# injun-baek/Video-Depth-Normal-v2

Measured on AMD Instinct MI355X. Metric: depth frames/sec at 518x518, ViT-L, higher is better.
Workload: dtype f16x3; 1 GPU; DepthAnythingV2(vitl) batch=8 518x518 streams/GPU, memory bank full (S=6); replicas per GPU; lanes=2, precision=f16x3, ranks=1, backend=none, attention_pv_products=1

## Files before the change

### include/vdn.h

```cpp
#ifndef VDN_H
#define VDN_H
#include <stddef.h>
#include <stdint.h>

#ifdef __cplusplus
extern "C" {
#endif

typedef void* vdn_stream;

enum vdn_status { VDN_OK = 0, VDN_EINVAL = -1, VDN_EUNSUPPORTED = -2, VDN_EALIGN = -3 };
enum vdn_dtype { VDN_F16 = 0, VDN_BF16 = 1, VDN_F32 = 2, VDN_NONE = 3 };
enum vdn_act { VDN_ACT_NONE = 0, VDN_ACT_GELU = 1, VDN_ACT_RELU = 2,
               VDN_ACT_SILU = 3  };
enum vdn_amode { VDN_A_PLAIN = 0, VDN_A_CONV3X3 = 1 };
enum vdn_store {
  VDN_ST_PLAIN = 0,
  VDN_ST_HEADS = 1,
  VDN_ST_CONVT = 2,
  VDN_ST_GEGLU = 3
};

typedef struct vdn_gemm_tuning {
  int force_bm;
  int p8;
  int no_splitk;
  int no_pipe;
  int splitk_p8;
  int cus;
  int splitk_occ;
  int splitk_max;
  int min_tiles;
  float f128, f192;
  int x8;
} vdn_gemm_tuning;
int vdn_gemm_get_tuning(vdn_gemm_tuning* out);

typedef struct vdn_gemm_desc {
  int32_t dt;
  int32_t M, N, K;
  const void* A;
  int32_t a_mode;
  int32_t lda;
  int32_t relu_a;
  int32_t cB, cH, cW, cC, cOH, cOW, cstride;
  const void* W;
  int32_t ldb;
  const float* bias;
  const float* rowadd;
  int32_t act;
  const float* gamma;
  const float* tab;
  int32_t tab_mod, tab_off;
  const void* res1;
  int32_t res1_dt, ldr1;
  const void* res2;
  int32_t res2_dt, ldr2;
  int32_t store;
  void* out;
  int32_t out_dt;
  int32_t ldc;
  int32_t row_group, row_skip;
  void* dst[3];
  int32_t nsplit, heads, tokens, tok_off, tpad;
  int32_t transposed[3];
  int32_t rope[3];
  const float* rope_cs;
  int32_t rope_mod;
  int32_t ck, cout;
  const void* zeros;
  const void* A_lo;
  const void* W_lo;
  void* out_lo;
  void* dst_lo[3];
  const void* res1_lo;
  const void* res2_lo;
  int32_t conv_korder;
  int32_t cu_hint;
  void* splitk_ws;
  int64_t splitk_ws_bytes;
  int32_t ksplit;
  void* dst8[3];
  const void* A8;
  const void* W8;
  void* out8;
  int32_t a_kt, w_kt, out_kt;
  int32_t x8_terms;
// ... 196 lines not shown
```

### video-depth-normal-v2_amd/csrc/common.hpp

```cpp
#pragma once
#include <hip/hip_runtime.h>
#include <stdint.h>
#include <type_traits>
#include "../../include/vdn.h"

typedef _Float16 f16x8 __attribute__((ext_vector_type(8)));
typedef _Float16 f16x4 __attribute__((ext_vector_type(4)));
typedef _Float16 f16x2 __attribute__((ext_vector_type(2)));
typedef __bf16 bf16x8 __attribute__((ext_vector_type(8)));
typedef __bf16 bf16x4 __attribute__((ext_vector_type(4)));
typedef __bf16 bf16x2 __attribute__((ext_vector_type(2)));
typedef float f32x2 __attribute__((ext_vector_type(2)));
typedef float f32x4 __attribute__((ext_vector_type(4)));
typedef float f32x16 __attribute__((ext_vector_type(16)));
typedef uint32_t u32x4 __attribute__((ext_vector_type(4)));
typedef uint32_t u32x2 __attribute__((ext_vector_type(2)));

#define VDN_CHECK_LAUNCH()                                   \
  do {                                                       \
    hipError_t e__ = hipGetLastError();                      \
    if (e__ != hipSuccess) return -(1000 + (int)e__);        \
  } while (0)

template <int DT> struct Half;
// ... 156 lines not shown
}
constexpr float VDN_LO8_SCALE = 1024.0f;
constexpr int VDN_LO8_E8M0 = 117;

typedef _Float16 f16x32 __attribute__((ext_vector_type(32)));
typedef unsigned u32x6 __attribute__((ext_vector_type(6)));
__device__ __forceinline__ int x6_scale_byte(const f16x32& hi) {
  typedef unsigned short u16x32 __attribute__((ext_vector_type(32)));
  typedef unsigned short u16x16 __attribute__((ext_vector_type(16)));
  typedef unsigned short u16x8 __attribute__((ext_vector_type(8)));
  typedef unsigned short u16x4 __attribute__((ext_vector_type(4)));
  typedef unsigned short u16x2 __attribute__((ext_vector_type(2)));
  const u16x32 b = __builtin_bit_cast(u16x32, hi) & (unsigned short)0x7FFF;
  const u16x16 m16 = __builtin_elementwise_max(b.lo, b.hi);
  const u16x8 m8 = __builtin_elementwise_max(m16.lo, m16.hi);
  const u16x4 m4 = __builtin_elementwise_max(m8.lo, m8.hi);
  const u16x2 m2 = __builtin_elementwise_max(m4.lo, m4.hi);
  const unsigned m = m2[0] > m2[1] ? m2[0] : m2[1];
  return (int)(m >> 10) + 108;
}
__device__ __forceinline__ void x6_store_half(uint8_t* dst, const f16x32& v, int scale_byte) {
  const u32x6 c = __builtin_amdgcn_cvt_scalef32_pk32_bf6_f16(v, __builtin_bit_cast(float, (unsigned)scale_byte << 23));
  *(u32x4*)dst = u32x4{c[0], c[1], c[2], c[3]};
  *(u32x4*)(dst + 16) = u32x4{c[4], c[5], (unsigned)scale_byte, 0u};
}
__host__ __device__ __forceinline__ int x6_col(int order, int h, int p) {
  return order == 1 ? 32 * (p >> 4) + 16 * ((p >> 3) & 1) + 8 * h + (p & 7)
       : order == 2 ? 32 * (p >> 4) + 8 * ((p >> 2) & 3) + 4 * h + (p & 3)
                    : 32 * h + p;
}

template <typename T>
__device__ __forceinline__ void store_half(T* hi, T* lo, size_t i, float v) {
  if (lo) { T a, b; split_rtz(v, a, b); hi[i] = a; lo[i] = b; }
  else hi[i] = (T)v;
}
template <typename T>
__device__ __forceinline__ void store_half_nearest(T* hi, T* lo, size_t i, float v) {
  const T a = (T)v;
  hi[i] = a;
  if (lo) lo[i] = (T)(v - (float)a);
}
template <typename T>
__device__ __forceinline__ float load_half(const T* hi, const T* lo, size_t i) {
  return lo ? (float)hi[i] + (float)lo[i] : (float)hi[i];
}

__device__ __forceinline__ int xcd_remap(int orig, int nwg) {
  const int xcd = orig & 7;
  const int q = nwg >> 3, r = nwg & 7;
  const int base = (xcd < r) ? xcd * (q + 1) : r * (q + 1) + (xcd - r) * q;
  return base + (orig >> 3);
}
```

### video-depth-normal-v2_amd/csrc/gemm.hip

```cpp
#include "common.hpp"
#include <stdlib.h>

namespace vdn_gemm_impl {
int launch_f16(const vdn_gemm_desc& d, hipStream_t s);
int launch_bf16(const vdn_gemm_desc& d, hipStream_t s);

static int env_int(const char* name, int dflt) {
  const char* e = getenv(name);
  return e ? atoi(e) : dflt;
}
static float env_float(const char* name, float dflt) {
  const char* e = getenv(name);
  return e ? (float)atof(e) : dflt;
}
static const vdn_gemm_tuning& tuning_defaults() {
  static const vdn_gemm_tuning t = [] {
    vdn_gemm_tuning v;
    v.force_bm = env_int("VDN_GEMM_BM", 0);
    v.p8 = env_int("VDN_GEMM_P8", 1);
    v.no_splitk = getenv("VDN_GEMM_NOSPLITK") != nullptr;
    v.no_pipe = getenv("VDN_GEMM_NOPIPE") != nullptr;
    v.splitk_p8 = env_int("VDN_SPLITK_P8", 0);
    v.cus = env_int("VDN_GEMM_CUS", 0);
    v.splitk_occ = env_int("VDN_SPLITK_OCC", 50);
    v.splitk_max = env_int("VDN_SPLITK_MAX", 8);
    v.min_tiles = env_int("VDN_GEMM_MIN_TILES", 96);
    v.f128 = env_float("VDN_GEMM_F128", 1.3f);
    v.f192 = env_float("VDN_GEMM_F192", 1.2f);
    v.x8 = env_int("VDN_GEMM_X8", 1);
    return v;
  }();
  return t;
}
const vdn_gemm_tuning& tuning(const vdn_gemm_desc& d) { return d.tuning ? *d.tuning : tuning_defaults(); }
}

extern "C" int vdn_gemm_get_tuning(vdn_gemm_tuning* out) {
  if (!out) return VDN_EINVAL;
  vdn_gemm_desc none = {};
  *out = vdn_gemm_impl::tuning(none);
  return VDN_OK;
}

extern "C" int vdn_gemm(const vdn_gemm_desc* dp, vdn_stream stream) {
  if (!dp) return VDN_EINVAL;
  const vdn_gemm_desc& d = *dp;
  if (d.M <= 0 || d.N <= 0 || d.K <= 0 || !d.A || !d.W || !d.zeros) return VDN_EINVAL;
  if (d.tuning) {
    const vdn_gemm_tuning& t = *d.tuning;
    if ((t.force_bm != 0 && t.force_bm != 128 && t.force_bm != 192 && t.force_bm != 256) || t.splitk_occ < 0 || t.splitk_max < 0 ||
        t.min_tiles < 0 || t.cus < 0 || t.cus > 256)
      return VDN_EINVAL;
  }
  if (d.dt != VDN_F16 && d.dt != VDN_BF16) return VDN_EUNSUPPORTED;
  if ((d.K & 7) || (d.ldb & 63) || d.ldb < d.K) return VDN_EALIGN;
  if (((uintptr_t)d.A & 15) || ((uintptr_t)d.W & 15) || ((uintptr_t)d.zeros & 15)) return VDN_EALIGN;
  if (d.subpix) {
    if (d.subpix != 1 || d.a_mode != VDN_A_CONV3X3 || d.store != VDN_ST_CONVT || !d.subpix_bias || d.bias || d.act || d.rowadd ||
        d.gamma || d.tab || d.res1 || d.res2 || d.relu_a || d.K != 4 * d.cC || d.ldb != d.K || d.conv_korder != 1 || d.cstride != 1)
      return VDN_EINVAL;
    if ((d.ck != 2 && d.ck != 4) || d.cout <= 0 || (d.cout & 255) || (d.cC & 63) || !d.A_lo || !d.W_lo || !d.out_lo ||
        d.out_dt != d.dt || d.A8 || d.W8)
      return VDN_EUNSUPPORTED;
    if (((uintptr_t)d.subpix_bias | (uintptr_t)d.out) & 15) return VDN_EALIGN;
  }
  if (d.a_mode == VDN_A_CONV3X3) {
    if ((d.cC & 7) || d.K != (d.subpix ? 4 : 9) * d.cC || d.M != d.cB * d.cOH * d.cOW) return VDN_EINVAL;
    if (d.conv_korder && ((d.cC & 63) || d.conv_korder != 1)) return VDN_EINVAL;
    if (d.cstride != 1 && d.cstride != 2) return VDN_EUNSUPPORTED;
    if (d.cOH != (d.cH + 2 - 3) / d.cstride + 1 || d.cOW != (d.cW + 2 - 3) / d.cstride + 1) return VDN_EINVAL;
  } else if (d.a_mode == VDN_A_PLAIN) {
    if ((d.lda & 7) || d.lda < d.K) return VDN_EALIGN;
  } else {
    return VDN_EUNSUPPORTED;
  }
  if (d.N & 3) return VDN_EALIGN;
  if (d.ksplit != 0 || d.splitk_ws_bytes < 0 || (d.splitk_ws == nullptr) != (d.splitk_ws_bytes == 0)) return VDN_EINVAL;
  if ((uintptr_t)d.splitk_ws & 15) return VDN_EALIGN;
  if (((uintptr_t)d.A_lo | (uintptr_t)d.W_lo | (uintptr_t)d.out_lo) & 15) return VDN_EALIGN;
  if (d.out_lo && (d.out_dt == VDN_F32 || !d.out)) return VDN_EINVAL;
  if ((d.res1 && (d.ldr1 & 3)) || (d.res2 && (d.ldr2 & 3))) return VDN_EALIGN;
  if (((uintptr_t)d.A8 | (uintptr_t)d.W8 | (uintptr_t)d.out8) & 15) return VDN_EALIGN;
  if ((d.A8 || d.W8) && (d.dt != VDN_F16 || d.a_mode != VDN_A_PLAIN || (d.K & 63) || (d.lda != d.K && !d.a_kt))) return VDN_EINVAL;
  if (d.out8 && (d.dt != VDN_F16 || d.store != VDN_ST_PLAIN || d.out_dt != VDN_F16 || d.act != VDN_ACT_GELU || d.N != d.ldc || (d.N & 63) || !d.A8 || !d.W8))
    return VDN_EINVAL;
  if ((d.a_kt || d.w_kt || d.out_kt || d.x8_terms) && (!d.A8 || !d.W8)) return VDN_EINVAL;
  if (d.A8 && d.W8 && ((!d.a_kt && (long)d.M * d.lda >= (1L << 31)) || (!d.w_kt && (long)d.N * d.ldb >= (1L << 31)) || d.M >= (1 << 25) || d.N >= (1 << 25)))
    return VDN_EUNSUPPORTED;
  if (d.x8_terms < 0 || d.x8_terms > 2) return VDN_EINVAL;
  if (d.out_kt && (d.store != VDN_ST_PLAIN || d.out_dt != VDN_F16 || d.ldc != d.N || (d.N & 63) || d.res1 || d.res2 || d.tab ||
                   d.rowadd || d.gamma || d.row_group > 0 || d.act == VDN_ACT_RELU)) return VDN_EINVAL;
  if (((uintptr_t)d.bias | (uintptr_t)d.gamma | (uintptr_t)d.tab | (uintptr_t)d.res1 | (uintptr_t)d.res2) & 7) return VDN_EALIGN;
  switch (d.store) {
    case VDN_ST_PLAIN:
      if (!d.out || d.ldc < d.N) return VDN_EINVAL;
      if ((d.ldc & 3) || ((uintptr_t)d.out & 15)) return VDN_EALIGN;
      break;
    case VDN_ST_GEGLU:
      if (!d.out || (d.N & 31) || d.ldc < d.N / 2 || (d.act && d.act != VDN_ACT_SILU) || d.gamma || d.res1 || d.res2 || d.tab || d.rowadd)
        return VDN_EINVAL;
      if ((d.ldc & 3) || ((uintptr_t)d.out & 15)) return VDN_EALIGN;
      break;
    case VDN_ST_CONVT:
      if (!d.out || d.ck <= 0 || d.cout <= 0 || d.N != d.ck * d.ck * d.cout || d.M != d.cB * d.cH * d.cW || d.res1 ||
// ... 22 lines not shown
```

### video-depth-normal-v2_amd/csrc/gemm_kernels.hpp

```cpp
#pragma once
#include "common.hpp"
#include <stdlib.h>
#include <type_traits>

namespace vdn_gemm_impl {

const vdn_gemm_tuning& tuning(const vdn_gemm_desc& d);

constexpr int BK = 64;


__device__ __forceinline__ void glds16(const void* src, void* dst) {
  __builtin_amdgcn_global_load_lds((const __attribute__((address_space(1))) void*)src, (__attribute__((address_space(3))) void*)dst,
                                   16, 0, 0);
}

__device__ __forceinline__ void tile_mn(int tile, int tiles_m, int tiles_n, int& tm_i, int& tn_i) {
  constexpr int GM = 4;
  const int per_group = GM * tiles_n;
  const int g = tile / per_group, r = tile - g * per_group;
  const int gm = (tiles_m - g * GM) < GM ? (tiles_m - g * GM) : GM;
  tn_i = r / gm;
  tm_i = g * GM + (r - tn_i * gm);
}
// ... 939 lines not shown
      const int cur = kt & 1;
      const char* sc = smem + cur * STAGE;
      const char* sn = smem + (cur ^ 1) * STAGE;
      read_a(sc, 1, a1h, a1l);
      mma(0, a0h, a0l, bch, bcl);
      stage_barrier();
      if (kt + 2 < nk) issue(cur, kt + 2);
      if (kt + 1 < nk) {
        read_b(sn, bnh, bnl);
        read_a(sn, 0, a0h, a0l);
      }
      mma(1, a1h, a1l, bch, bcl);
    };
    int kt = 0;
    for (; kt + 1 < nk; kt += 2) {
      pstep(kt, b0h, b0l, b1h, b1l);
      pstep(kt + 1, b1h, b1l, b0h, b0l);
    }
    if (kt < nk) pstep(kt, b0h, b0l, b1h, b1l);
    stage_barrier();
  }

  epilogue_x3<DT, TMW, STORE>(acc, p, slice, m0 + wm * (BM / 2), n0 + wn * 64, lane);
}

template <int DT, int AMODE, int STORE, int BM>
__global__ __launch_bounds__(512) void gemm_x3_p8_kernel(const vdn_gemm_desc p) {
  using H = Half<DT>;
  using V8 = typename H::V8;
  using T = typename H::T;
  static_assert(BM == 256 || BM == 192, "A sub-halves of 64 or 48 rows");
  constexpr int BN = 256, BK3 = 32;
  constexpr int A_TILE = BM * 64, W_TILE = BN * 64;
  constexpr int STAGE = 2 * A_TILE + 2 * W_TILE;
  constexpr int TQ = BM / 64;
  constexpr bool CONV = (AMODE == 1 || AMODE == 2);
  constexpr bool RELU_A = (AMODE == 2 || AMODE == 3);
  extern __shared__ __attribute__((aligned(16))) char smem[];

  const int tid = threadIdx.x, lane = tid & 63;
  const int wave = __builtin_amdgcn_readfirstlane(tid >> 6);
  const int tiles_n = (p.N + BN - 1) / BN;
  const int tiles_m = (p.M + BM - 1) / BM;
  const int ntiles = tiles_m * tiles_n;
  constexpr bool SPLITK = STORE == VDN_STX_SPLITK;
  const int slice = SPLITK ? (int)blockIdx.x / ntiles : 0;
  const bool persistent = !SPLITK && (int)gridDim.x < ntiles;
  for (int it = 0;; ++it) {
  int tile;
  if constexpr (SPLITK) {
    if (it) break;
    tile = xcd_remap((int)blockIdx.x - slice * ntiles, ntiles);
  } else if (persistent) {
    const int xcd = blockIdx.x & 7, q8 = ntiles >> 3, r8 = ntiles & 7;
    const int base = xcd < r8 ? xcd * (q8 + 1) : r8 * (q8 + 1) + (xcd - r8) * q8;
    const int idx = (int)(blockIdx.x >> 3) + it * (int)(gridDim.x >> 3);
    if (idx >= q8 + (xcd < r8 ? 1 : 0)) break;
    tile = base + idx;
  } else {
    if (it) break;
    tile = xcd_remap(blockIdx.x, ntiles);
  }
  int tm_i, tn_i;
  tile_mn(tile, tiles_m, tiles_n, tm_i, tn_i);
  constexpr bool SUBPIX = STORE == VDN_STX_SUBPIX;
  unsigned sp_taps = 0;
  int sp_lg = 0;
  const int m0 = tm_i * BM, n0 = SUBPIX ? subpix_tile(tn_i, p, sp_taps, sp_lg) : tn_i * BN;
  const int wm = wave >> 2, wn = wave & 3;

  const int kt0s = SPLITK ? slice * ((((AMODE == 1 || AMODE == 2) ? p.ldb / BK3 : p.K / BK3) + p.ksplit - 1) / p.ksplit) : 0;
  const int lr = lane >> 2;
  const int chunk = (lane & 3) ^ ((0 - (lane >> 4)) & 3);
  const int a_li = (BM == 256 || wave < 4) ? wave : 4 + ((wave - 4) >> 1);
  const bool a_both = BM == 256 || wave < 4;
  const int a_plane = a_both ? 0 : (wave & 1);
  const int pa[2] = {(a_li / TQ) * 2 * TQ + a_li % TQ, (a_li / TQ) * 2 * TQ + TQ + a_li % TQ};
  const int pw[2] = {4 * (wave >> 1) + (wave & 1), 4 * (wave >> 1) + (wave & 1) + 2};
  APiece<T, CONV> a_pc[2];
#pragma unroll
  for (int i = 0; i < 2; ++i) a_pc[i].setup(m0 + pa[i] * 16 + lr, chunk * 8, p);
  const char* zeros = (const char*)p.zeros;
  const ptrdiff_t a_delta = (const char*)p.A_lo - (const char*)p.A;
  const ptrdiff_t w_delta = (const char*)p.W_lo - (const char*)p.W;
  const char* ap[2];
  const char* wp[2];
#pragma unroll
  for (int i = 0; i < 2; ++i) {
    int n = n0 + (vdn_pair8<STORE> ? (pw[i] >> 2) * 64 + pair8_col(pw[i] & 3, lr) : pw[i] * 16 + lr);
    n = n < p.N ? n : p.N - 1;
    wp[i] = (const char*)((const T*)p.W + (size_t)n * p.ldb + chunk * 8);
    ap[i] = (const char*)(a_pc[i].base + chunk * 8);
  }
  auto issue = [&](auto uc, int buf, int kt) {
    constexpr int u = decltype(uc)::value;
    char* s0 = smem + buf * STAGE;
    if constexpr (u == 0 || u == 3) {
      constexpr int i = u == 0 ? 0 : 1;
      char* dst = s0 + pa[i] * 1024;
      if constexpr (CONV) {
        bool ok;
        const char* src = a_pc[i].src(kstep_decode<BK3, SUBPIX>(kt + kt0s, p, sp_taps, sp_lg), chunk * 8, p, ok);
        if (a_both) {
          glds16(ok ? src : zeros, dst);
          glds16(ok ? src + a_delta : zeros, dst + A_TILE);
        } else {
          glds16(ok ? src + (a_plane ? a_delta : 0) : zeros, dst + a_plane * A_TILE);
        }
      } else {
        if (a_both) {
          glds16(ap[i], dst);
// ... 305 lines not shown
```

### video-depth-normal-v2_amd/csrc/gemm_x8.hip

```cpp
#include "gemm_kernels.hpp"

namespace vdn_gemm_impl {

typedef int i32x8 __attribute__((ext_vector_type(8)));

constexpr int X8_BN = 256;
constexpr int X8_WH = 256 * 64;
#ifndef VDN_X8_NSLOT
#define VDN_X8_NSLOT 5
#endif
#ifndef VDN_X8_ABL
#define VDN_X8_ABL 0
#endif
constexpr int X8_NSLOT = VDN_X8_NSLOT;
constexpr int x8_unit(int bm) { return bm * 64 + X8_WH; }
constexpr int X8_L = X8_NSLOT - 1;
constexpr int x8_pc(int ph, bool four) {
  const int a = four ? 2 : 1, w = 2;
  return a + w;
}
constexpr int x8_inflight(int newest, int k, bool four) {
  int n = 0;
  for (int t = 0; t < k; ++t) n += x8_pc((newest - t) & 3, four);
  return n;
}

template <int STORE, bool PAIR, int X8_BM>
__global__ __launch_bounds__(512) void gemm_x8_kernel(const vdn_gemm_desc p) {
  using H = Half<VDN_F16>;
  using V8 = H::V8;
  static_assert(X8_BM == 256 || X8_BM == 192, "two wave groups of 4 or 3 blocks of 32 rows");
  constexpr int X8_H = X8_BM * 64, X8_U = x8_unit(X8_BM), NI = X8_BM / 64, AP = X8_BM / 16;
  extern __shared__ __attribute__((aligned(16))) char smem[];

  const int tid = threadIdx.x, lane = tid & 63;
  const int wave = __builtin_amdgcn_readfirstlane(tid >> 6);
  const int tiles_n = (p.N + X8_BN - 1) / X8_BN, tiles_m = (p.M + X8_BM - 1) / X8_BM;
  int tm_i, tn_i;
  tile_mn(xcd_remap(blockIdx.x, tiles_m * tiles_n), tiles_m, tiles_n, tm_i, tn_i);
  const int m0 = tm_i * X8_BM, n0 = tn_i * X8_BN;
  const int wm = wave >> 2, wn = wave & 3;
  const int r = lane & 31, h = lane >> 5;

  const int lr = lane >> 2, chunk = (lane & 3) ^ ((0 - (lane >> 4)) & 3);
  const size_t a_rs = p.a_kt ? 64 : (size_t)p.lda * 2, a_kts = p.a_kt ? (size_t)p.M * 64 : 64;
  const size_t w_rs = p.w_kt ? 64 : (size_t)p.ldb * 2, w_kts = p.w_kt ? (size_t)p.N * 64 : 64;
  const size_t a8_rs = p.a_kt ? 64 : (size_t)p.lda, a8_kts = p.a_kt ? (size_t)p.M * 64 : 64;
  const size_t w8_rs = p.w_kt ? 64 : (size_t)p.ldb, w8_kts = p.w_kt ? (size_t)p.N * 64 : 64;
  unsigned ah_o[2], wh_o[2], a8_o[2], w8_o[2];
#pragma unroll
  for (int i = 0; i < 2; ++i) {
    const int lrw = PAIR ? ((lr & 3) | ((lr & 4) << 1) | ((lr & 8) >> 1)) : lr;
    int m = m0 + (wave + 8 * i) * 16 + lr, n = n0 + (wave + 8 * i) * 16 + lrw;
    m = m < p.M ? m : p.M - 1;
    n = n < p.N ? n : p.N - 1;
    ah_o[i] = (unsigned)(m * a_rs) + chunk * 16;
    wh_o[i] = (unsigned)(n * w_rs) + chunk * 16;
    a8_o[i] = (unsigned)(m * a8_rs) + chunk * 16;
    w8_o[i] = (unsigned)(n * w8_rs) + chunk * 16;
  }
  const char* Ah = (const char*)p.A;
  const char* Wh = (const char*)p.W;
  const char* A8v = (const char*)p.A8;
  const char* W8v = (const char*)p.W8;
  const size_t a8l = (size_t)p.M * p.K, w8l = (size_t)p.N * p.ldb;
  auto issue = [&](int slab, auto phc, int slot) {
    constexpr int ph = decltype(phc)::value;
    if constexpr (VDN_X8_ABL & 2) return;
    char* ua = smem + slot * X8_U;
    char* uw = ua + X8_H;
    const char *ba, *bw;
    if constexpr (ph < 2) {
      ba = Ah + (size_t)(2 * slab + ph) * a_kts;
      bw = Wh + (size_t)(2 * slab + ph) * w_kts;
    } else {
      ba = A8v + (ph == 2 ? a8l : 0) + (size_t)slab * a8_kts;
      bw = W8v + (ph == 2 ? 0 : w8l) + (size_t)slab * w8_kts;
    }
#pragma unroll
    for (int i = 0; i < 2; ++i) {
      unsigned oa = ph < 2 ? ah_o[i] : a8_o[i], ow = ph < 2 ? wh_o[i] : w8_o[i];
      asm volatile("" : "+v"(oa), "+v"(ow));
      if (AP == 16 || wave + 8 * i < AP) glds16(ba + oa, ua + (wave + 8 * i) * 1024);
      glds16(bw + ow, uw + (wave + 8 * i) * 1024);
    }
  };
  const bool four = AP == 16 || wave < 4;
#define X8_WAIT(NEWPH, K)                                                                                     \
  do {                                                                                                        \
    if (four) asm volatile("s_waitcnt vmcnt(%0)" ::"n"(x8_inflight((NEWPH), (K), true)) : "memory");          \
    else asm volatile("s_waitcnt vmcnt(%0)" ::"n"(x8_inflight((NEWPH), (K), false)) : "memory");              \
  } while (0)

  const int swz = (0 - (r >> 2)) & 3;
  const int a_off0 = (wm * (X8_BM / 2) + r) * 64 + ((h ^ swz) << 4);
  const int w_off0 = X8_H + (wn * 64 + r) * 64 + ((h ^ swz) << 4);
  const int a8_off0 = (wm * (X8_BM / 2) + r) * 64 + (((2 * h) ^ swz) << 4);
  const int w8_off0 = X8_H + (wn * 64 + r) * 64 + (((2 * h) ^ swz) << 4);
  auto rd8 = [&](const char* u, int off) {
    const u32x4 a0 = *(const u32x4*)(u + off), a1 = *(const u32x4*)(u + (off ^ 16));
    i32x8 v;
#pragma unroll
    for (int e = 0; e < 4; ++e) { v[e] = (int)a0[e]; v[4 + e] = (int)a1[e]; }
    return v;
  };

  f32x16 acc[NI][2];
#pragma unroll
  for (int i = 0; i < NI; ++i)
#pragma unroll
    for (int j = 0; j < 2; ++j)
#pragma unroll
      for (int e = 0; e < 16; ++e) acc[i][j][e] = 0.f;

  const int m_alo = p.x8_terms == 1 ? 0 : -1, m_wlo = p.x8_terms == 2 ? 0 : -1;
  V8 hw[2][2] = {}, ha[2][NI] = {};
  i32x8 cw[2] = {}, ca[NI] = {};
  auto reads = [&](auto phc, int slot) {
    constexpr int ph = decltype(phc)::value;
    if constexpr (VDN_X8_ABL & 4) return;
    const char* u = smem + slot * X8_U;
    if constexpr (ph < 2) {
#pragma unroll
      for (int ks = 0; ks < 2; ++ks) {
#pragma unroll
        for (int j = 0; j < 2; ++j) hw[ks][j] = *(const V8*)(u + (w_off0 ^ (ks << 5)) + j * 2048);
#pragma unroll
        for (int i = 0; i < NI; ++i) ha[ks][i] = *(const V8*)(u + (a_off0 ^ (ks << 5)) + i * 2048);
      }
    } else {
#pragma unroll
      for (int j = 0; j < 2; ++j) cw[j] = rd8(u + j * 2048, w8_off0);
#pragma unroll
      for (int i = 0; i < NI; ++i) ca[i] = rd8(u + i * 2048, a8_off0);
    }
  };
  auto mfmas = [&](auto phc) {
    constexpr int ph = decltype(phc)::value;
    if constexpr (VDN_X8_ABL & 1) {
      if constexpr (ph < 2) { for (int ks = 0; ks < 2; ++ks) { for (int j = 0; j < 2; ++j) asm volatile("" ::"v"(hw[ks][j])); for (int i = 0; i < NI; ++i) asm volatile("" ::"v"(ha[ks][i])); } }
      else { for (int j = 0; j < 2; ++j) asm volatile("" ::"v"(cw[j])); for (int i = 0; i < NI; ++i) asm volatile("" ::"v"(ca[i])); }
      return;
    }
    __builtin_amdgcn_s_setprio(1);
    if constexpr (ph < 2) {
#pragma unroll
      for (int ks = 0; ks < 2; ++ks)
#pragma unroll
        for (int i = 0; i < NI; ++i)
#pragma unroll
          for (int j = 0; j < 2; ++j) {
            acc[i][j] = H::mfma32(hw[ks][j], ha[ks][i], acc[i][j]);
            if (j == 1) __builtin_amdgcn_sched_barrier(0);
          }
    } else {
#pragma unroll
      for (int i = 0; i < NI; ++i)
#pragma unroll
        for (int j = 0; j < 2; ++j) {
          const int sw = cw[j][6], sa = ca[i][6];
          if constexpr (ph == 2) acc[i][j] = __builtin_amdgcn_mfma_scale_f32_32x32x64_f8f6f4(cw[j], ca[i], acc[i][j], 3, 3, 0, sw, 0, sa & m_alo);
          else acc[i][j] = __builtin_amdgcn_mfma_scale_f32_32x32x64_f8f6f4(cw[j], ca[i], acc[i][j], 3, 3, 0, sw & m_wlo, 0, sa);
          if (j == 1) __builtin_amdgcn_sched_barrier(0);
        }
    }
    __builtin_amdgcn_s_setprio(0);
  };

  const int nslab = p.K >> 6;
  const int nunits = 4 * nslab;
#if VDN_X8_ABL & 8
  const unsigned long long st_c0 = __builtin_amdgcn_s_memtime(), st_r0 = __builtin_amdgcn_s_memrealtime();
#endif
  constexpr std::integral_constant<int, 0> P0{};
  constexpr std::integral_constant<int, 1> P1{};
  constexpr std::integral_constant<int, 2> P2{};
  constexpr std::integral_constant<int, 3> P3{};
  int rd_slot = 0, wr_slot = X8_L % X8_NSLOT;
  auto next = [](int s) { return s + 1 == X8_NSLOT ? 0 : s + 1; };

  {
    int s = 0;
    auto pro = [&](int n, auto phc) {
      if (n < X8_L && n < nunits) { issue(n >> 2, phc, s); s = next(s); }
    };
    pro(0, P0); pro(1, P1); pro(2, P2); pro(3, P3);
    if constexpr (X8_L > 4) pro(4, P0);
  }
  if (nunits >= X8_L) X8_WAIT((X8_L - 1) & 3, X8_L - 1);
  else asm volatile("s_waitcnt vmcnt(0)" ::: "memory");
  __builtin_amdgcn_s_barrier();
  if (wm == 1) __builtin_amdgcn_s_barrier();

#define X8_PHASE(PC, PH)                                                                    \
  do {                                                                                      \
    reads(PC, rd_slot);                                                                     \
    X8_ISSUE(PH);                                                                           \
    X8_WAIT(((PH) + X8_L) & 3, X8_L - 1);                                                   \
    asm volatile("s_waitcnt lgkmcnt(0)" ::: "memory");                                      \
    __builtin_amdgcn_s_barrier();                                                           \
    __builtin_amdgcn_sched_barrier(0);                                                      \
    mfmas(PC);                                                                              \
    __builtin_amdgcn_sched_barrier(0);                                                      \
    __builtin_amdgcn_s_barrier();                                                           \
    rd_slot = next(rd_slot);                                                                \
    wr_slot = next(wr_slot);                                                                \
  } while (0)
#define X8_ISSUE(PH) issue(s + ((PH) + X8_L) / 4, std::integral_constant<int, ((PH) + X8_L) & 3>{}, wr_slot)
  int s = 0;
  for (; 4 * s + 3 + X8_L <= nunits - 1; ++s) {
    X8_PHASE(P0, 0);
    X8_PHASE(P1, 1);
    X8_PHASE(P2, 2);
    X8_PHASE(P3, 3);
  }
  static_assert(X8_L == 4, "the tail below is written for a lead of one slab");
#define X8_TAIL(PC, LEFT)                                                                   \
  do {                                                                                      \
    reads(PC, rd_slot);                                                                     \
    if constexpr ((LEFT) > 0) X8_WAIT(3, (LEFT));                                           \
    else asm volatile("s_waitcnt vmcnt(0)" ::: "memory");                                   \
    asm volatile("s_waitcnt lgkmcnt(0)" ::: "memory");                                      \
    __builtin_amdgcn_s_barrier();                                                           \
    __builtin_amdgcn_sched_barrier(0);                                                      \
    mfmas(PC);                                                                              \
    __builtin_amdgcn_sched_barrier(0);                                                      \
    __builtin_amdgcn_s_barrier();                                                           \
    rd_slot = next(rd_slot);                                                                \
  } while (0)
  for (; s < nslab; ++s) {
    X8_TAIL(P0, 2);
    X8_TAIL(P1, 1);
    X8_TAIL(P2, 0);
    X8_TAIL(P3, 0);
  }
#undef X8_TAIL
#undef X8_ISSUE
#undef X8_PHASE
  if (wm == 0) __builtin_amdgcn_s_barrier();
  __builtin_amdgcn_sched_barrier(0);
#if VDN_X8_ABL & 8
  if (p.splitk_ws && tid == 0 && (blockIdx.x % 37) == 0) {
    unsigned long long* dbg = (unsigned long long*)p.splitk_ws + (blockIdx.x / 37) * 2;
    dbg[0] = __builtin_amdgcn_s_memtime() - st_c0;
    dbg[1] = __builtin_amdgcn_s_memrealtime() - st_r0;
  }
#endif

  const int mw = m0 + wm * (X8_BM / 2), nw = n0 + wn * 64;
  const f32x4 z4 = {0.f, 0.f, 0.f, 0.f}, o4 = {1.f, 1.f, 1.f, 1.f};
  if constexpr (PAIR) {
    f32x4 bias8[2][2][2];
#pragma unroll
    for (int j = 0; j < 2; ++j)
#pragma unroll
      for (int u = 0; u < 2; ++u)
#pragma unroll
        for (int q = 0; q < 2; ++q) {
          const int n = nw + 32 * j + 16 * u + 8 * h + 4 * q;
          bias8[j][u][q] = (p.bias && n < p.N) ? *(const f32x4*)(p.bias + n) : z4;
        }
    if (STORE == VDN_STX_FC1 && p.out8) {
#pragma unroll
      for (int i = 0; i < NI; ++i) {
        const int m = mw + 32 * i + r;
        f16x32 hv, lv;
#pragma unroll
        for (int j = 0; j < 2; ++j)
#pragma unroll
          for (int u = 0; u < 2; ++u) {
            const f32x4 g0 = gelu4(f32x4{acc[i][j][8 * u], acc[i][j][8 * u + 1], acc[i][j][8 * u + 2], acc[i][j][8 * u + 3]} + bias8[j][u][0]);
            const f32x4 g1 = gelu4(f32x4{acc[i][j][8 * u + 4], acc[i][j][8 * u + 5], acc[i][j][8 * u + 6], acc[i][j][8 * u + 7]} + bias8[j][u][1]);
            V8 hh, ll;
#pragma unroll
            for (int e = 0; e < 4; e += 2) {
              _Float16 h0, h1, l0, l1;
              split2_rtz(g0[e], g0[e + 1], h0, h1, l0, l1);
              hh[e] = h0; hh[e + 1] = h1; ll[e] = l0; ll[e + 1] = l1;
              split2_rtz(g1[e], g1[e + 1], h0, h1, l0, l1);
              hh[4 + e] = h0; hh[5 + e] = h1; ll[4 + e] = l0; ll[5 + e] = l1;
            }
#pragma unroll
            for (int e = 0; e < 8; ++e) { hv[16 * j + 8 * u + e] = hh[e]; lv[16 * j + 8 * u + e] = ll[e]; }
            const int n = nw + 32 * j + 16 * u + 8 * h;
            if (m < p.M && n < p.N) {
              const size_t o = p.out_kt ? ((size_t)(n >> 5) * p.M + m) * 32 + (n & 31) : (size_t)m * p.ldc + n;
              *(V8*)((_Float16*)p.out + o) = hh;
              if (p.out_lo) *(V8*)((_Float16*)p.out_lo + o) = ll;
            }
          }
        if (m < p.M && nw < p.N) {
          const int sb = x6_scale_byte(hv);
          uint8_t* d8 = (uint8_t*)p.out8 + (p.out_kt ? ((size_t)(nw >> 6) * p.M + m) * 64 : (size_t)m * p.ldc + nw) + 32 * h;
          x6_store_half(d8, hv, sb);
          x6_store_half(d8 + (size_t)p.M * p.ldc, lv, sb - 10);
        }
      }
    } else if ((STORE == VDN_STX_HEADS || STORE == VDN_ST_HEADS) && nw < p.N && !p.transposed[nw / (p.heads * 64)] && p.dst8[nw / (p.heads * 64)]) {
      const int hc = p.heads * 64, split = nw / hc, head = (nw - split * hc) >> 6;
      _Float16* dst = (_Float16*)p.dst[split];
      _Float16* dlo = (_Float16*)p.dst_lo[split];
      if (STORE == VDN_ST_HEADS && p.rope[split]) {
        f32x4 cs[2][2][4];
        auto fetch = [&](int i, f32x4 (&d)[2][4]) {
          const int m = mw + 32 * i + r, mc = m < p.M ? m : p.M - 1;
          const int tl = mc - (mc / p.tokens) * p.tokens;
          const float* t = p.rope_cs + (size_t)(tl % p.rope_mod) * 64 + 16 * h;
#pragma unroll
          for (int j = 0; j < 2; ++j)
#pragma unroll
            for (int q = 0; q < 4; ++q) d[j][q] = *(const f32x4*)(t + 32 * j + 4 * q);
        };
        fetch(0, cs[0]);
#pragma unroll
// ... 69 lines not shown
          }
        u32x4 bh[2], bl[2];
#pragma unroll
        for (int u = 0; u < 2; ++u)
#pragma unroll
          for (int w = 0; w < 2; ++w) {
            const auto sh = __builtin_amdgcn_permlane32_swap(hi8[0][u][w], hi8[1][u][w], false, false);
            const auto sl = __builtin_amdgcn_permlane32_swap(lo8[0][u][w], lo8[1][u][w], false, false);
            bh[u][w] = sh[0]; bh[u][2 + w] = sh[1];
            bl[u][w] = sl[0]; bl[u][2 + w] = sl[1];
          }
        if (m < p.M) {
          uint8_t* d8 = (uint8_t*)p.dst8[split] + row * 128 + 32 * h;
          *(u32x4*)d8 = bh[0];
          *(u32x4*)(d8 + 16) = bh[1];
          *(u32x4*)(d8 + 64) = bl[0];
          *(u32x4*)(d8 + 80) = bl[1];
        }
      }
    } else {
#pragma unroll
      for (int i = 0; i < NI; ++i)
#pragma unroll
        for (int j = 0; j < 2; ++j)
#pragma unroll
          for (int u = 0; u < 2; ++u) {
            const f32x4 a0 = {acc[i][j][8 * u], acc[i][j][8 * u + 1], acc[i][j][8 * u + 2], acc[i][j][8 * u + 3]};
            const f32x4 a1 = {acc[i][j][8 * u + 4], acc[i][j][8 * u + 5], acc[i][j][8 * u + 6], acc[i][j][8 * u + 7]};
            emit8<VDN_F16, STORE == VDN_ST_HEADS ? VDN_STX_HEADS : STORE>(p, mw + 32 * i + r, nw + 32 * j + 16 * u + 8 * h, a0, a1, bias8[j][u][0],
                                                                              bias8[j][u][1]);
          }
    }
  } else if constexpr (STORE == VDN_STX_RES) {
    f32x4 bias4[2][4], gam4[2][4];
#pragma unroll
    for (int j = 0; j < 2; ++j)
#pragma unroll
      for (int g = 0; g < 4; ++g) {
        const int n = nw + 32 * j + 8 * g + 4 * h;
        bias4[j][g] = (p.bias && n < p.N) ? *(const f32x4*)(p.bias + n) : z4;
        gam4[j][g] = (p.gamma && n < p.N) ? *(const f32x4*)(p.gamma + n) : o4;
      }
    f32x4 res[2][2][4];
    auto fetch = [&](int i, f32x4 (&dst)[2][4]) {
      const int m = mw + 32 * i + r;
#pragma unroll
      for (int j = 0; j < 2; ++j)
#pragma unroll
        for (int g = 0; g < 4; ++g) {
          const int n = nw + 32 * j + 8 * g + 4 * h;
          dst[j][g] = (m < p.M && n < p.N) ? *(const f32x4*)((const float*)p.res1 + (size_t)m * p.ldr1 + n) : z4;
        }
    };
    fetch(0, res[0]);
#pragma unroll
    for (int i = 0; i < NI; ++i) {
      if (i + 1 < NI) fetch(i + 1, res[(i + 1) & 1]);
      const int m = mw + 32 * i + r;
#pragma unroll
      for (int j = 0; j < 2; ++j)
#pragma unroll
        for (int g = 0; g < 4; ++g) {
          const int n = nw + 32 * j + 8 * g + 4 * h;
          const f32x4 a = {acc[i][j][4 * g], acc[i][j][4 * g + 1], acc[i][j][4 * g + 2], acc[i][j][4 * g + 3]};
          if (m < p.M && n < p.N) *(f32x4*)((float*)p.out + (size_t)m * p.ldc + n) = (a + bias4[j][g]) * gam4[j][g] + res[i & 1][j][g];
        }
    }
  } else {
    f32x4 bias4[2][4], gam4[2][4];
#pragma unroll
    for (int j = 0; j < 2; ++j)
#pragma unroll
      for (int g = 0; g < 4; ++g) {
        const int n = nw + 32 * j + 8 * g + 4 * h;
        bias4[j][g] = (p.bias && n < p.N) ? *(const f32x4*)(p.bias + n) : z4;
        gam4[j][g] = (p.gamma && n < p.N) ? *(const f32x4*)(p.gamma + n) : o4;
      }
#pragma unroll
    for (int j = 0; j < 2; ++j)
#pragma unroll
      for (int g = 0; g < 4; ++g) {
        const int n = nw + 32 * j + 8 * g + 4 * h;
        const int gb = (g + 2) & 3;
#pragma unroll
        for (int i = 0; i < NI; ++i) {
          const f32x4 a = {acc[i][j][4 * g], acc[i][j][4 * g + 1], acc[i][j][4 * g + 2], acc[i][j][4 * g + 3]};
          const f32x4 b = {acc[i][j][4 * gb], acc[i][j][4 * gb + 1], acc[i][j][4 * gb + 2], acc[i][j][4 * gb + 3]};
          emit4<VDN_F16, STORE>(p, mw + 32 * i + r, n, a, b, bias4[j][g], bias4[j][gb], gam4[j][g]);
        }
      }
  }
}
#undef X8_WAIT

template <int BM>
static int x8_launch(const vdn_gemm_desc& d, hipStream_t s) {
  const int tiles = ((d.M + BM - 1) / BM) * ((d.N + X8_BN - 1) / X8_BN);
  const dim3 g(tiles), b(512);
  constexpr int LDS = X8_NSLOT * x8_unit(BM);
#define VDN_X8(ST, PAIR)                                                                                               \
  do {                                                                                                                   \
    static const hipError_t attr = hipFuncSetAttribute((const void*)gemm_x8_kernel<ST, PAIR, BM>,                        \
                                                       hipFuncAttributeMaxDynamicSharedMemorySize, LDS);       \
    if (attr != hipSuccess) return -(1000 + (int)attr);                                                                  \
    hipLaunchKernelGGL((gemm_x8_kernel<ST, PAIR, BM>), g, b, LDS, s, d);                                                 \
  } while (0)
  int fl = epi_flavour(d);
  const bool a8 = !(d.N & 7) && !(d.ldc & 7) && !((uintptr_t)d.out & 15) && !((uintptr_t)d.out_lo & 15) && !((uintptr_t)d.out8 & 7);
  if (d.out8 && !(a8 && fl == VDN_STX_FC1 && !(d.N & 63))) return VDN_EUNSUPPORTED;
  if (!a8 && fl != VDN_STX_RES && fl != VDN_STX_HEADS) fl = d.store;
  if (fl == VDN_STX_RESHALF1 || fl == VDN_STX_RESHALF2) fl = d.store;
  switch (fl) {
    case VDN_STX_FC1: VDN_X8(VDN_STX_FC1, true); break;
    case VDN_STX_HALF: VDN_X8(VDN_STX_HALF, true); break;
    case VDN_STX_HEADS: VDN_X8(VDN_STX_HEADS, true); break;
    case VDN_STX_RES: VDN_X8(VDN_STX_RES, false); break;
    case VDN_ST_GEGLU: VDN_X8(VDN_ST_GEGLU, false); break;
    case VDN_ST_HEADS: {
      bool pair = a8 && d.nsplit >= 1 && d.rope_cs && !((uintptr_t)d.rope_cs & 15);
      for (int i = 0; i < d.nsplit && pair; ++i)
        pair = d.dst[i] && (d.transposed[i] ? !d.rope[i] : d.dst8[i] != nullptr);
      if (pair) VDN_X8(VDN_ST_HEADS, true);
      else VDN_X8(VDN_ST_HEADS, false);
      break;
    }
    default: VDN_X8(VDN_ST_PLAIN, false); break;
  }
#undef VDN_X8
  VDN_CHECK_LAUNCH();
  return VDN_OK;
}

int x8_entry(const vdn_gemm_desc& d, hipStream_t s) {
  const vdn_gemm_tuning& tu = tuning(d);
  const int cus = tu.cus > 0 ? tu.cus : (d.cu_hint > 0 && d.cu_hint <= 256 ? d.cu_hint : 256);
  const long tn = (d.N + X8_BN - 1) / X8_BN;
  auto cost = [&](int bm, double f) { const long t = (long)((d.M + bm - 1) / bm) * tn; return (double)((t + cus - 1) / cus) * bm * f; };
  int bm = tu.force_bm == 192 || tu.force_bm == 256 ? tu.force_bm : (cost(192, 1.08) < cost(256, 1.0) ? 192 : 256);
  return bm == 192 ? x8_launch<192>(d, s) : x8_launch<256>(d, s);
}

}
```

### video-depth-normal-v2_amd/vdn/_abi.py

```python
from __future__ import annotations

import ctypes as C
import os

PKG = os.path.dirname(os.path.dirname(os.path.abspath(__file__)))
LIB_PATH = os.environ.get("VDN_LIB") or os.path.join(PKG, "lib", "libvdn_hip.so")

F16, BF16, F32, NONE = 0, 1, 2, 3
ACT_NONE, ACT_GELU, ACT_RELU, ACT_SILU = 0, 1, 2, 3
OUT_NONE, OUT_RELU, OUT_SIGMOID = 0, 1, 2
A_PLAIN, A_CONV3X3 = 0, 1
ST_PLAIN, ST_HEADS, ST_CONVT, ST_GEGLU = 0, 1, 2, 3
EVAL_DEPTH, EVAL_DISP = 0, 1
EVAL_TGM_ROWS, EVAL_TGM_FRAMES = 0, 1
PACK_LINEAR, PACK_CONV3X3, PACK_CONV3X3_TAPS, PACK_CONVT, PACK_GEGLU, PACK_ROPE = 0, 1, 2, 3, 4, 5

i32, vp, fp = C.c_int32, C.c_void_p, C.c_void_p


class GemmDesc(C.Structure):
    _fields_ = [
        ("dt", i32), ("M", i32), ("N", i32), ("K", i32),
        ("A", vp), ("a_mode", i32), ("lda", i32), ("relu_a", i32),
        ("cB", i32), ("cH", i32), ("cW", i32), ("cC", i32), ("cOH", i32), ("cOW", i32), ("cstride", i32),
        ("W", vp), ("ldb", i32),
        ("bias", fp), ("rowadd", fp), ("act", i32), ("gamma", fp), ("tab", fp), ("tab_mod", i32), ("tab_off", i32),
        ("res1", vp), ("res1_dt", i32), ("ldr1", i32),
        ("res2", vp), ("res2_dt", i32), ("ldr2", i32),
        ("store", i32), ("out", vp), ("out_dt", i32), ("ldc", i32), ("row_group", i32), ("row_skip", i32),
        ("dst", vp * 3), ("nsplit", i32), ("heads", i32), ("tokens", i32), ("tok_off", i32), ("tpad", i32),
        ("transposed", i32 * 3), ("rope", i32 * 3),
        ("rope_cs", fp), ("rope_mod", i32),
        ("ck", i32), ("cout", i32), ("zeros", vp),
        ("A_lo", vp), ("W_lo", vp), ("out_lo", vp), ("dst_lo", vp * 3), ("res1_lo", vp), ("res2_lo", vp),
        ("conv_korder", i32), ("cu_hint", i32),
        ("splitk_ws", vp), ("splitk_ws_bytes", C.c_int64), ("ksplit", i32),
        ("dst8", vp * 3),
        ("A8", vp), ("W8", vp), ("out8", vp),
        ("a_kt", i32), ("w_kt", i32), ("out_kt", i32), ("x8_terms", i32),
        ("tuning", vp),
        ("subpix", i32), ("subpix_bias", fp),
    ]


class GemmTuning(C.Structure):
    _fields_ = [("force_bm", i32), ("p8", i32), ("no_splitk", i32), ("no_pipe", i32), ("splitk_p8", i32),
                ("cus", i32), ("splitk_occ", i32), ("splitk_max", i32), ("min_tiles", i32), ("f128", C.c_float),
                ("f192", C.c_float), ("x8", i32)]


class VdnError(RuntimeError):
    pass


def _load():
    if not os.path.exists(LIB_PATH):
        raise ImportError(
            f"{LIB_PATH} not found: the HIP extension is required (there is no CPU fallback). "
            f"Build it with `python __graft_entry__.py build` (hipcc --offload-arch=gfx950).")
    try:
        return C.CDLL(LIB_PATH)
    except OSError as e:
        raise ImportError(f"cannot load {LIB_PATH}: {e}. Rebuild with `python __graft_entry__.py build`.") from e


lib = _load()

EXPORTS = {
    "vdn_gemm": (C.c_int, [C.POINTER(GemmDesc), vp]),
    "vdn_gemm_get_tuning": (C.c_int, [C.POINTER(GemmTuning)]),
    "vdn_layernorm": (C.c_int, [vp, C.c_int, C.c_int, C.c_int, fp, fp, C.c_float, fp, C.c_float, fp, C.c_int, C.c_int,
                                C.c_int, vp, vp, C.c_int, fp, vp, C.c_int, vp]),
    "vdn_flash_attn": (C.c_int, [C.c_int, vp, vp, vp, vp, vp, vp, vp, vp, vp, vp, vp, C.c_int, C.c_int, C.c_int, C.c_int, C.c_int,
                                 C.c_int, C.c_int, C.c_float, C.c_int, vp]),
    "vdn_temporal_attn": (C.c_int, [C.c_int, vp, vp, vp, vp, C.c_int, C.c_int, C.c_int, C.c_int, C.c_int, C.c_float, fp, vp]),
    "vdn_groupnorm": (C.c_int, [C.c_int, vp, vp, vp, vp, C.c_int, C.c_int, C.c_int, C.c_int, fp, fp, C.c_float, fp,
                                C.c_int, vp]),
    "vdn_upsample_bilinear": (C.c_int, [C.c_int, vp, vp, vp, vp, C.c_int, C.c_int, C.c_int, C.c_int, C.c_int, C.c_int, vp]),
    "vdn_upsample_bilinear_f32": (C.c_int, [fp, fp, C.c_int, C.c_int, C.c_int, C.c_int, C.c_int, C.c_int, vp]),
    "vdn_patchify": (C.c_int, [C.c_int, fp, vp, vp, C.c_int, C.c_int, C.c_int, C.c_int, vp]),
    "vdn_fill_row": (C.c_int, [fp, fp, C.c_int, C.c_int, C.c_int, C.c_int, vp]),
    "vdn_bicubic": (C.c_int, [fp, fp, C.c_int, C.c_int, C.c_int, C.c_int, C.c_int, C.c_float, C.c_float, vp]),
    "vdn_preprocess": (C.c_int, [vp, C.c_int, C.c_int, C.c_int, C.c_int, fp, C.c_int, C.c_int, C.POINTER(C.c_float), C.POINTER(C.c_float), vp]),
    "vdn_add_vec": (C.c_int, [fp, fp, C.c_float, fp, C.c_int, C.c_int, vp]),
    "vdn_head_out": (C.c_int, [C.c_int, vp, vp, fp, C.c_float, fp, C.c_int, C.c_int, C.c_int, vp]),
    "vdn_depth_tail": (C.c_int, [C.c_int, fp, C.c_int, C.c_int, C.c_int, C.c_int, vp, vp, C.c_int, fp, fp, C.c_float, fp,
                                 C.c_int, C.c_int, C.c_int, vp]),
    "vdn_head_out_act": (C.c_int, [C.c_int, vp, vp, fp, C.c_float, fp, C.c_int, C.c_int, C.c_int, C.c_float, vp]),
    "vdn_depth_tail_act": (C.c_int, [C.c_int, fp, C.c_int, C.c_int, C.c_int, C.c_int, vp, vp, C.c_int, fp, fp, C.c_float, fp,
                                     C.c_int, C.c_int, C.c_int, C.c_float, vp]),
    "vdn_depth_to_points": (C.c_int, [fp, vp, C.c_int, C.c_int, C.c_double, C.c_double, vp, vp, vp]),
    "vdn_oc1_combine": (C.c_int, [fp, fp, fp, C.c_int, C.c_int, C.c_int, C.c_int, C.c_int, C.c_int, vp]),
    "vdn_pack_rows": (C.c_int, [C.c_int, C.c_int, C.c_int, C.c_int]),
    "vdn_pack_ldb": (C.c_int, [C.c_int, C.c_int, C.c_int, C.c_int]),
    "vdn_pack_weight": (C.c_int, [C.c_int, C.c_int, fp, C.c_int, C.c_int, C.c_int, vp, vp, C.c_int, vp]),
    "vdn_pack_bias": (C.c_int, [C.c_int, fp, C.c_int, C.c_int, C.c_int, fp, vp]),
    "vdn_pack_x8": (C.c_int, [vp, vp, C.c_int, C.c_int, vp, vp, C.c_int, C.c_int, vp]),
    "vdn_pack_x8_f32": (C.c_int, [fp, C.c_int, C.c_int, vp, vp, vp]),
    "vdn_gemm_workspace_bytes": (C.c_size_t, [C.POINTER(GemmDesc)]),
    "vdn_groupnorm_workspace_bytes": (C.c_size_t, [C.c_int, C.c_int, C.c_int]),
    "vdn_mask_down1": (C.c_int, [fp, fp, C.c_int, C.c_int, C.c_int, C.c_int, C.c_int, fp, vp]),
# ... 114 lines not shown
```

Measured before the change: 291.1 frames/s.

## Add persistent x8 GEMM kernel that prefetches the next tile during the epilogue

Adds a persistent variant of the x8 (split-precision) GEMM kernel. Each workgroup walks tiles in XCD-grouped order and issues the next tile's prologue loads before running the current tile's epilogue. It launches one workgroup per CU when the tile count is at least twice the CU count, and applies to every epilogue except the residual and heads stores. The aim is to hide prologue load latency and launch tail behind epilogue work, at the cost of more register pressure and a fixed one-WG-per-CU grid.

Result: no change. 291.4 frames/s, median of 2 (+0.1%).

```diff
diff --git a/include/vdn.h b/include/vdn.h
--- a/include/vdn.h
+++ b/include/vdn.h
@@ -33,6 +33,7 @@
   int min_tiles;
   float f128, f192;
   int x8;
+  int persistent;
 } vdn_gemm_tuning;
 int vdn_gemm_get_tuning(vdn_gemm_tuning* out);
 
diff --git a/video-depth-normal-v2_amd/csrc/common.hpp b/video-depth-normal-v2_amd/csrc/common.hpp
--- a/video-depth-normal-v2_amd/csrc/common.hpp
+++ b/video-depth-normal-v2_amd/csrc/common.hpp
@@ -232,3 +232,10 @@
   const int base = (xcd < r) ? xcd * (q + 1) : r * (q + 1) + (xcd - r) * q;
   return base + (orig >> 3);
 }
+__device__ __forceinline__ int xcd_walk(int bid, int nwg, int it, int ntiles) {
+  const int xcd = bid & 7;
+  const int q = ntiles >> 3, r = ntiles & 7;
+  const int base = (xcd < r) ? xcd * (q + 1) : r * (q + 1) + (xcd - r) * q;
+  const int idx = (bid >> 3) + it * (nwg >> 3);
+  return idx < q + (xcd < r ? 1 : 0) ? base + idx : -1;
+}
diff --git a/video-depth-normal-v2_amd/csrc/gemm.hip b/video-depth-normal-v2_amd/csrc/gemm.hip
--- a/video-depth-normal-v2_amd/csrc/gemm.hip
+++ b/video-depth-normal-v2_amd/csrc/gemm.hip
@@ -28,6 +28,7 @@
     v.f128 = env_float("VDN_GEMM_F128", 1.3f);
     v.f192 = env_float("VDN_GEMM_F192", 1.2f);
     v.x8 = env_int("VDN_GEMM_X8", 1);
+    v.persistent = env_int("VDN_X8_PERSISTENT", 2);
     return v;
   }();
   return t;
@@ -49,7 +50,7 @@
   if (d.tuning) {
     const vdn_gemm_tuning& t = *d.tuning;
     if ((t.force_bm != 0 && t.force_bm != 128 && t.force_bm != 192 && t.force_bm != 256) || t.splitk_occ < 0 || t.splitk_max < 0 ||
-        t.min_tiles < 0 || t.cus < 0 || t.cus > 256)
+        t.min_tiles < 0 || t.cus < 0 || t.cus > 256 || t.persistent < 0 || t.persistent > 2)
       return VDN_EINVAL;
   }
   if (d.dt != VDN_F16 && d.dt != VDN_BF16) return VDN_EUNSUPPORTED;
diff --git a/video-depth-normal-v2_amd/csrc/gemm_kernels.hpp b/video-depth-normal-v2_amd/csrc/gemm_kernels.hpp
--- a/video-depth-normal-v2_amd/csrc/gemm_kernels.hpp
+++ b/video-depth-normal-v2_amd/csrc/gemm_kernels.hpp
@@ -1015,11 +1015,8 @@
     if (it) break;
     tile = xcd_remap((int)blockIdx.x - slice * ntiles, ntiles);
   } else if (persistent) {
-    const int xcd = blockIdx.x & 7, q8 = ntiles >> 3, r8 = ntiles & 7;
-    const int base = xcd < r8 ? xcd * (q8 + 1) : r8 * (q8 + 1) + (xcd - r8) * q8;
-    const int idx = (int)(blockIdx.x >> 3) + it * (int)(gridDim.x >> 3);
-    if (idx >= q8 + (xcd < r8 ? 1 : 0)) break;
-    tile = base + idx;
+    tile = xcd_walk(blockIdx.x, gridDim.x, it, ntiles);
+    if (tile < 0) break;
   } else {
     if (it) break;
     tile = xcd_remap(blockIdx.x, ntiles);
diff --git a/video-depth-normal-v2_amd/csrc/gemm_x8.hip b/video-depth-normal-v2_amd/csrc/gemm_x8.hip
--- a/video-depth-normal-v2_amd/csrc/gemm_x8.hip
+++ b/video-depth-normal-v2_amd/csrc/gemm_x8.hip
@@ -25,7 +25,7 @@
   return n;
 }
 
-template <int STORE, bool PAIR, int X8_BM>
+template <int STORE, bool PAIR, int X8_BM, bool PERSIST>
 __global__ __launch_bounds__(512) void gemm_x8_kernel(const vdn_gemm_desc p) {
   using H = Half<VDN_F16>;
   using V8 = H::V8;
@@ -36,18 +36,25 @@
   const int tid = threadIdx.x, lane = tid & 63;
   const int wave = __builtin_amdgcn_readfirstlane(tid >> 6);
   const int tiles_n = (p.N + X8_BN - 1) / X8_BN, tiles_m = (p.M + X8_BM - 1) / X8_BM;
+  const int ntiles = tiles_m * tiles_n;
   int tm_i, tn_i;
-  tile_mn(xcd_remap(blockIdx.x, tiles_m * tiles_n), tiles_m, tiles_n, tm_i, tn_i);
-  const int m0 = tm_i * X8_BM, n0 = tn_i * X8_BN;
+  tile_mn(PERSIST ? xcd_walk(blockIdx.x, gridDim.x, 0, ntiles) : xcd_remap(blockIdx.x, ntiles), tiles_m, tiles_n, tm_i, tn_i);
+  int m0 = tm_i * X8_BM, n0 = tn_i * X8_BN;
   const int wm = wave >> 2, wn = wave & 3;
   const int r = lane & 31, h = lane >> 5;
 
-  const int lr = lane >> 2, chunk = (lane & 3) ^ ((0 - (lane >> 4)) & 3);
+  auto fresh = [](int v) {
+    if constexpr (PERSIST) asm volatile("" : "+v"(v));
+    return v;
+  };
+  const int ln0 = fresh(lane);
+  const int lr0 = ln0 >> 2, chunk0 = (ln0 & 3) ^ ((0 - (ln0 >> 4)) & 3);
   const size_t a_rs = p.a_kt ? 64 : (size_t)p.lda * 2, a_kts = p.a_kt ? (size_t)p.M * 64 : 64;
   const size_t w_rs = p.w_kt ? 64 : (size_t)p.ldb * 2, w_kts = p.w_kt ? (size_t)p.N * 64 : 64;
   const size_t a8_rs = p.a_kt ? 64 : (size_t)p.lda, a8_kts = p.a_kt ? (size_t)p.M * 64 : 64;
   const size_t w8_rs = p.w_kt ? 64 : (size_t)p.ldb, w8_kts = p.w_kt ? (size_t)p.N * 64 : 64;
   unsigned ah_o[2], wh_o[2], a8_o[2], w8_o[2];
+  auto place = [&](int m0, int n0, int lr, int chunk) {
 #pragma unroll
   for (int i = 0; i < 2; ++i) {
     const int lrw = PAIR ? ((lr & 3) | ((lr & 4) << 1) | ((lr & 8) >> 1)) : lr;
@@ -59,6 +66,12 @@
     a8_o[i] = (unsigned)(m * a8_rs) + chunk * 16;
     w8_o[i] = (unsigned)(n * w8_rs) + chunk * 16;
   }
+  };
+  place(m0, n0, lr0, chunk0);
+  auto place_again = [&](int m0, int n0) {
+    const int ln = fresh(lane);
+    place(m0, n0, ln >> 2, (ln & 3) ^ ((0 - (ln >> 4)) & 3));
+  };
   const char* Ah = (const char*)p.A;
   const char* Wh = (const char*)p.W;
   const char* A8v = (const char*)p.A8;
@@ -92,11 +105,15 @@
     else asm volatile("s_waitcnt vmcnt(%0)" ::"n"(x8_inflight((NEWPH), (K), false)) : "memory");              \
   } while (0)
 
-  const int swz = (0 - (r >> 2)) & 3;
-  const int a_off0 = (wm * (X8_BM / 2) + r) * 64 + ((h ^ swz) << 4);
-  const int w_off0 = X8_H + (wn * 64 + r) * 64 + ((h ^ swz) << 4);
-  const int a8_off0 = (wm * (X8_BM / 2) + r) * 64 + (((2 * h) ^ swz) << 4);
-  const int w8_off0 = X8_H + (wn * 64 + r) * 64 + (((2 * h) ^ swz) << 4);
+  int a_off0, w_off0, a8_off0, w8_off0;
+  auto frag_offsets = [&](int r, int h) {
+    const int swz = (0 - (r >> 2)) & 3;
+    a_off0 = (wm * (X8_BM / 2) + r) * 64 + ((h ^ swz) << 4);
+    w_off0 = X8_H + (wn * 64 + r) * 64 + ((h ^ swz) << 4);
+    a8_off0 = (wm * (X8_BM / 2) + r) * 64 + (((2 * h) ^ swz) << 4);
+    w8_off0 = X8_H + (wn * 64 + r) * 64 + (((2 * h) ^ swz) << 4);
+  };
+  frag_offsets(r, h);
   auto rd8 = [&](const char* u, int off) {
     const u32x4 a0 = *(const u32x4*)(u + off), a1 = *(const u32x4*)(u + (off ^ 16));
     i32x8 v;
@@ -106,12 +123,15 @@
   };
 
   f32x16 acc[NI][2];
+  auto zero_acc = [&]() {
 #pragma unroll
   for (int i = 0; i < NI; ++i)
 #pragma unroll
     for (int j = 0; j < 2; ++j)
 #pragma unroll
       for (int e = 0; e < 16; ++e) acc[i][j][e] = 0.f;
+  };
+  zero_acc();
 
   const int m_alo = p.x8_terms == 1 ? 0 : -1, m_wlo = p.x8_terms == 2 ? 0 : -1;
   V8 hw[2][2] = {}, ha[2][NI] = {};
@@ -179,15 +199,41 @@
   int rd_slot = 0, wr_slot = X8_L % X8_NSLOT;
   auto next = [](int s) { return s + 1 == X8_NSLOT ? 0 : s + 1; };
 
-  {
+  auto prologue = [&]() {
     int s = 0;
     auto pro = [&](int n, auto phc) {
       if (n < X8_L && n < nunits) { issue(n >> 2, phc, s); s = next(s); }
     };
     pro(0, P0); pro(1, P1); pro(2, P2); pro(3, P3);
     if constexpr (X8_L > 4) pro(4, P0);
-  }
-  if (nunits >= X8_L) X8_WAIT((X8_L - 1) & 3, X8_L - 1);
+  };
+  prologue();
+  int ntile = -1;
+  auto prefetch = [&](int it) {
+    ntile = xcd_walk(blockIdx.x, gridDim.x, it + 1, ntiles);
+    if (ntile >= 0) {
+      int ti, tj;
+      tile_mn(ntile, tiles_m, tiles_n, ti, tj);
+      place_again(ti * X8_BM, tj * X8_BN);
+      prologue();
+    }
+    __builtin_amdgcn_sched_barrier(0);
+  };
+  auto held = [](auto& v) { asm volatile("" : "+v"(v)); };
+
+  for (int it = 0;; ++it) {
+  if (PERSIST && it > 0) {
+    int t = ntile;
+    asm volatile("" : "+s"(t));
+    tile_mn(t, tiles_m, tiles_n, tm_i, tn_i);
+    m0 = tm_i * X8_BM, n0 = tn_i * X8_BN;
+    place_again(m0, n0);
+    const int lf = fresh(lane);
+    frag_offsets(lf & 31, lf >> 5);
+    zero_acc();
+    rd_slot = 0, wr_slot = X8_L % X8_NSLOT;
+  }
+  if ((!PERSIST || it == 0) && nunits >= X8_L) X8_WAIT((X8_L - 1) & 3, X8_L - 1);
   else asm volatile("s_waitcnt vmcnt(0)" ::: "memory");
   __builtin_amdgcn_s_barrier();
   if (wm == 1) __builtin_amdgcn_s_barrier();
@@ -247,6 +293,7 @@
   }
 #endif
 
+  const int le = fresh(lane), r = le & 31, h = le >> 5;
   const int mw = m0 + wm * (X8_BM / 2), nw = n0 + wn * 64;
   const f32x4 z4 = {0.f, 0.f, 0.f, 0.f}, o4 = {1.f, 1.f, 1.f, 1.f};
   if constexpr (PAIR) {
@@ -260,6 +307,13 @@
           const int n = nw + 32 * j + 16 * u + 8 * h + 4 * q;
           bias8[j][u][q] = (p.bias && n < p.N) ? *(const f32x4*)(p.bias + n) : z4;
         }
+    if constexpr (PERSIST) {
+#pragma unroll
+      for (int j = 0; j < 2; ++j)
+#pragma unroll
+        for (int u = 0; u < 2; ++u) { held(bias8[j][u][0]); held(bias8[j][u][1]); }
+      prefetch(it);
+    }
     if (STORE == VDN_STX_FC1 && p.out8) {
 #pragma unroll
       for (int i = 0; i < NI; ++i) {
@@ -435,6 +489,7 @@
           dst[j][g] = (m < p.M && n < p.N) ? *(const f32x4*)((const float*)p.res1 + (size_t)m * p.ldr1 + n) : z4;
         }
     };
+    static_assert(!PERSIST, "no persistent form of the residual epilogue: it spills (x8_can_persist)");
     fetch(0, res[0]);
 #pragma unroll
     for (int i = 0; i < NI; ++i) {
@@ -459,6 +514,13 @@
         bias4[j][g] = (p.bias && n < p.N) ? *(const f32x4*)(p.bias + n) : z4;
         gam4[j][g] = (p.gamma && n < p.N) ? *(const f32x4*)(p.gamma + n) : o4;
       }
+    if constexpr (PERSIST) {
+#pragma unroll
+      for (int j = 0; j < 2; ++j)
+#pragma unroll
+        for (int g = 0; g < 4; ++g) { held(bias4[j][g]); held(gam4[j][g]); }
+      prefetch(it);
+    }
 #pragma unroll
     for (int j = 0; j < 2; ++j)
 #pragma unroll
@@ -473,20 +535,45 @@
         }
       }
   }
+  if (!PERSIST || ntile < 0) break;
+  }
 }
 #undef X8_WAIT
+
+static int x8_device_cus() {
+  static const int n = [] {
+    int dev = 0;
+    hipDeviceProp_t prop;
+    if (hipGetDevice(&dev) != hipSuccess || hipGetDeviceProperties(&prop, dev) != hipSuccess) return 256;
+    return prop.multiProcessorCount;
+  }();
+  return n;
+}
+
+constexpr bool x8_can_persist(int st) { return st != VDN_STX_RES && st != VDN_ST_HEADS; }
+
+template <int ST, bool PAIR, int BM, bool PERSIST>
+static int x8_go(const vdn_gemm_desc& d, int grid, hipStream_t s) {
+  constexpr int LDS = X8_NSLOT * x8_unit(BM);
+  static const hipError_t attr = hipFuncSetAttribute((const void*)gemm_x8_kernel<ST, PAIR, BM, PERSIST>,
+                                                     hipFuncAttributeMaxDynamicSharedMemorySize, LDS);
+  if (attr != hipSuccess) return -(1000 + (int)attr);
+  hipLaunchKernelGGL((gemm_x8_kernel<ST, PAIR, BM, PERSIST>), dim3(grid), dim3(512), LDS, s, d);
+  return VDN_OK;
+}
 
 template <int BM>
 static int x8_launch(const vdn_gemm_desc& d, hipStream_t s) {
   const int tiles = ((d.M + BM - 1) / BM) * ((d.N + X8_BN - 1) / X8_BN);
-  const dim3 g(tiles), b(512);
-  constexpr int LDS = X8_NSLOT * x8_unit(BM);
+  const vdn_gemm_tuning& tu = tuning(d);
+  const int cus = (tu.cus > 0 ? tu.cus : x8_device_cus()) & ~7;
+  const bool persist = cus > 0 && (tu.persistent == 1 ? tiles > cus : tu.persistent == 2 && tiles >= 2 * cus);
 #define VDN_X8(ST, PAIR)                                                                                               \
   do {                                                                                                                   \
-    static const hipError_t attr = hipFuncSetAttribute((const void*)gemm_x8_kernel<ST, PAIR, BM>,                        \
-                                                       hipFuncAttributeMaxDynamicSharedMemorySize, LDS);       \
-    if (attr != hipSuccess) return -(1000 + (int)attr);                                                                  \
-    hipLaunchKernelGGL((gemm_x8_kernel<ST, PAIR, BM>), g, b, LDS, s, d);                                                 \
+    int rc;                                                                                                              \
+    if constexpr (x8_can_persist(ST)) rc = persist ? x8_go<ST, PAIR, BM, true>(d, cus, s) : x8_go<ST, PAIR, BM, false>(d, tiles, s); \
+    else rc = x8_go<ST, PAIR, BM, false>(d, tiles, s);                                                                   \
+    if (rc != VDN_OK) return rc;                                                                                         \
   } while (0)
   int fl = epi_flavour(d);
   const bool a8 = !(d.N & 7) && !(d.ldc & 7) && !((uintptr_t)d.out & 15) && !((uintptr_t)d.out_lo & 15) && !((uintptr_t)d.out8 & 7);
diff --git a/video-depth-normal-v2_amd/vdn/_abi.py b/video-depth-normal-v2_amd/vdn/_abi.py
--- a/video-depth-normal-v2_amd/vdn/_abi.py
+++ b/video-depth-normal-v2_amd/vdn/_abi.py
@@ -46,7 +46,7 @@
 class GemmTuning(C.Structure):
     _fields_ = [("force_bm", i32), ("p8", i32), ("no_splitk", i32), ("no_pipe", i32), ("splitk_p8", i32),
                 ("cus", i32), ("splitk_occ", i32), ("splitk_max", i32), ("min_tiles", i32), ("f128", C.c_float),
-                ("f192", C.c_float), ("x8", i32)]
+                ("f192", C.c_float), ("x8", i32), ("persistent", i32)]
 
 
 class VdnError(RuntimeError):
```
